# ParthaEth/GIF

Hardware: NVIDIA H100
Metric: G+D train step images/sec @256x256 bs32/GPU (higher is better)
Workload: dtype bf16x3 error-compensated tensor-core contraction (two-term bf16 operands, 3 MMAs per slice), f32 accumulate/storage

## Files before the change

### gif_b200/csrc/conv_wgrad_tc.cu

```cuda
#include <stdlib.h>

#include "tc_common.cuh"

namespace gifb200 {
namespace {

constexpr int kWgStages = 4;
constexpr int kPix = 32;
constexpr int kWgConsumerWarps = 8;
constexpr int kWgThreads = 32 * kWgConsumerWarps + 32;

struct WgParams {
    int B, Hs, Ws, Cs, Hb, Wb, Cb;
    int k, pad, s2, flip;
    int pw;
    int mr_s, mr_b;
    long long units;
    int splits;
    long long stride_t, stride_cs, stride_cb;
    long long part_stride;
};

constexpr int kHaloRows = kPix + 2;

template <int KW, int BLOCK_N, bool HALO = false, bool X3 = false, int AC = 4>
struct WgSmem {
    static constexpr int kRowBytes = X3 ? 64 : 128;
    static constexpr int kChunkBytes = kPix * kRowBytes;
    static constexpr int kHaloChunkBytes = 5120;
    static constexpr int kPlanes = X3 ? 2 : 1;
    static constexpr int kBChunks = BLOCK_N / 32;
    static constexpr int kAPlaneBytes = AC * kChunkBytes;
    static constexpr int kABytes = kPlanes * kAPlaneBytes;
    static constexpr int kBPlaneBytes = kBChunks * (HALO ? kHaloChunkBytes : kChunkBytes);
    static constexpr int kBBytesPerTap = kPlanes * kBPlaneBytes;
    static constexpr int kStages = HALO ? 5 : kWgStages;
    static constexpr int kStageBytes = HALO ? kABytes + kBBytesPerTap : kABytes + KW * kBBytesPerTap;
    static constexpr int kTxBytes = HALO ? kABytes + kPlanes * kBChunks * kHaloRows * kRowBytes : kStageBytes;
    static constexpr int kBarrierOffset = (kStages * kStageBytes + 1023) / 1024 * 1024;
    static constexpr int kDynamic = kBarrierOffset + 128 + 1024;
    static_assert(!(HALO && X3), "the halo tile is an fp32-only layout");
};

__device__ __forceinline__ uint32_t sw128_off(int row, int ch) {
    return static_cast<uint32_t>(row * 128 + ((((ch >> 2) ^ row) & 7) << 4) + (ch & 3) * 4);
}

template <int KW, int BLOCK_N, bool STACK, bool HALO, bool X3, int AC>
__global__ void __launch_bounds__(kWgThreads, 1) wgrad_tc_kernel(const __grid_constant__ CUtensorMap map_s,
                                                                 const __grid_constant__ CUtensorMap map_s2,
                                                                 const __grid_constant__ CUtensorMap map_b,
                                                                 const __grid_constant__ CUtensorMap map_b2,
                                                                 float* __restrict__ part, const WgParams p) {
    using L = WgSmem<KW, BLOCK_N, HALO, X3, AC>;
    constexpr int kM = 32 * AC;
    constexpr int kChunkBytes = L::kChunkBytes;
    constexpr int kHaloChunkBytes = L::kHaloChunkBytes;
    constexpr int kNStages = L::kStages;
    extern __shared__ uint8_t smem_raw[];
    uint8_t* smem = reinterpret_cast<uint8_t*>((reinterpret_cast<uintptr_t>(smem_raw) + 1023) & ~static_cast<uintptr_t>(1023));
    uint64_t* full_bar = reinterpret_cast<uint64_t*>(smem + L::kBarrierOffset);
    uint64_t* empty_bar = full_bar + kNStages;
    const int warp = threadIdx.x >> 5, lane = threadIdx.x & 31;

    const int ms = blockIdx.x;
    const int nb = blockIdx.y;
    const int kh = STACK ? 0 : blockIdx.z / p.splits, split = STACK ? blockIdx.z : blockIdx.z % p.splits;
    const long long per = (p.units + p.splits - 1) / p.splits;
    const long long u0 = split * per;
    const long long u1 = u0 + per < p.units ? u0 + per : p.units;
    const int iters = u1 > u0 ? static_cast<int>(u1 - u0) : 0;

    if (warp == kWgConsumerWarps && lane == 0) {
        asm volatile("prefetch.tensormap [%0];" ::"l"(&map_s) : "memory");
        asm volatile("prefetch.tensormap [%0];" ::"l"(&map_b) : "memory");
        if (X3) {
            asm volatile("prefetch.tensormap [%0];" ::"l"(&map_s2) : "memory");
            asm volatile("prefetch.tensormap [%0];" ::"l"(&map_b2) : "memory");
        }
        for (int s = 0; s < kNStages; ++s) { mbar_init(&full_bar[s], 1); mbar_init(&empty_bar[s], kWgConsumerWarps); }
        asm volatile("fence.mbarrier_init.release.cluster;" ::: "memory");
        asm volatile("fence.proxy.async.shared::cta;" ::: "memory");
    }
    __syncthreads();

    if (warp == kWgConsumerWarps) {
        if (lane == 0) {
            const int rows = kPix / p.pw;
            const int segs = p.Ws / p.pw;
            const int row_bytes = p.pw * L::kRowBytes;
            int stage = 0;
            uint32_t ph = 0;
            for (int it = 0; it < iters; ++it) {
                const long long u = u0 + it;
                mbar_wait(&empty_bar[stage], ph ^ 1);
                uint8_t* a_dst = smem + stage * L::kStageBytes;
                uint8_t* b_dst = a_dst + L::kABytes;
                mbar_expect_tx(&full_bar[stage], L::kTxBytes);
                for (int r = 0; r < rows; ++r) {
                    long long grow;
                    int x0;
                    if (rows == 1) { grow = u / segs; x0 = static_cast<int>(u % segs) * kPix; }
                    else { grow = u * rows + r; x0 = 0; }
                    const int n = static_cast<int>(grow / p.Hs), y = static_cast<int>(grow % p.Hs);
#pragma unroll
                    for (int pl = 0; pl < L::kPlanes; ++pl) {
                        const CUtensorMap* ms_ = pl ? &map_s2 : &map_s;
                        const CUtensorMap* mb_ = pl ? &map_b2 : &map_b;
                        uint8_t* a_pl = a_dst + pl * L::kAPlaneBytes;
                        if (r == 0 || !p.mr_s) {
                            for (int c = 0; c < AC; ++c) {
                                if (STACK)
                                    tma_load_4d(a_pl + c * kChunkBytes + r * row_bytes, ms_, &full_bar[stage], 0, x0,
                                                y + 1 - (c < 3 ? c : 2), n);
                                else if (AC == 2)
                                    tma_load_4d(a_pl + c * kChunkBytes + r * row_bytes, ms_, &full_bar[stage],
                                                c * 32 < p.Cs ? c * 32 : 0, x0, y, n);
                                else
                                    tma_load_4d(a_pl + c * kChunkBytes + r * row_bytes, ms_, &full_bar[stage], ms * 128 + c * 32, x0, y, n);
                            }
                        }
                        if (HALO) {
                            for (int c = 0; c < L::kBChunks; ++c)
                                tma_load_4d(b_dst + pl * L::kBPlaneBytes + c * kHaloChunkBytes, mb_, &full_bar[stage],
                                            nb * BLOCK_N + c * 32, x0 - 1, y + (STACK ? 0 : kh - p.pad), n);
                            continue;
                        }
                        if (r != 0 && p.mr_b) continue;
                        for (int kw = 0; kw < KW; ++kw)
                            for (int c = 0; c < L::kBChunks; ++c) {
                                uint8_t* dst = b_dst + kw * L::kBBytesPerTap + pl * L::kBPlaneBytes + c * kChunkBytes + r * row_bytes;
                                const int ch = nb * BLOCK_N + c * 32;
                                if (STACK)
                                    tma_load_4d(dst, mb_, &full_bar[stage], ch, x0 + kw - 1, y, n);
                                else if (!p.s2)
                                    tma_load_4d(dst, mb_, &full_bar[stage], ch, x0 + kw - p.pad, y + kh - p.pad, n);
                                else
                                    tma_load_5d(dst, mb_, &full_bar[stage], ch, kw & 1, x0 + (kw >> 1), 2 * y + kh, n);
                            }
                    }
                }
                if (++stage == kNStages) { stage = 0; ph ^= 1; }
            }
        }
        return;
    }

    float* pbase = part + split * p.part_stride;
    const int g = lane >> 2, tq = lane & 3;
    if (X3) {
        const int wg = warp >> 2, wq = warp & 3;
        constexpr int kSlices = AC == 4 ? kPix / 16 : 1;
        constexpr int kAcc = BLOCK_N / 2;
        float acc[KW][kAcc];
#pragma unroll
        for (int kw = 0; kw < KW; ++kw)
#pragma unroll
            for (int i = 0; i < kAcc; ++i) acc[kw][i] = 0.f;
        int stage = 0, prev = -1;
        uint32_t ph = 0;
        for (int it = 0; it < iters; ++it) {
            mbar_wait(&full_bar[stage], ph);
            const uint32_t a_addr = smem_u32(smem + stage * L::kStageBytes);
            const uint32_t a_row = AC == 4 ? wg * 2 * kChunkBytes : 0;
            const uint64_t adesc = make_smem_desc(a_addr + a_row, kChunkBytes, 512, 2);
            const uint64_t adesc_lo = make_smem_desc(a_addr + L::kAPlaneBytes + a_row, kChunkBytes, 512, 2);
            wgmma_fence();
#pragma unroll
            for (int kw = 0; kw < KW; ++kw) {
                fence_regs<kAcc>(acc[kw]);
                const uint32_t b_addr = a_addr + L::kABytes + kw * L::kBBytesPerTap;
                const uint64_t bdesc = make_smem_desc(b_addr, kChunkBytes, 512, 2);
                const uint64_t bdesc_lo = make_smem_desc(b_addr + L::kBPlaneBytes, kChunkBytes, 512, 2);
#pragma unroll
                for (int jj = 0; jj < kSlices; ++jj) {
                    const int j = AC == 4 ? jj : wg;
                    wgmma_bf16<BLOCK_N>(acc[kw], adesc_lo + 64 * j, bdesc + 64 * j, 1, Trans<1>());
                    wgmma_bf16<BLOCK_N>(acc[kw], adesc + 64 * j, bdesc_lo + 64 * j, 1, Trans<1>());
                    wgmma_bf16<BLOCK_N>(acc[kw], adesc + 64 * j, bdesc + 64 * j, 1, Trans<1>());
                }
            }
            wgmma_commit();
#pragma unroll
            for (int kw = 0; kw < KW; ++kw) fence_regs<kAcc>(acc[kw]);
            wgmma_wait<1>();
            if (prev >= 0 && lane == 0) mbar_arrive(&empty_bar[prev]);
            prev = stage;
            if (++stage == kNStages) { stage = 0; ph ^= 1; }
        }
        wgmma_wait<0>();
#pragma unroll
        for (int kw = 0; kw < KW; ++kw) fence_regs<kAcc>(acc[kw]);
        if constexpr (AC == 2) {
            static_assert(KW * kAcc * 128 * 4 <= kNStages * L::kStageBytes, "exchange buffer exceeds the stage ring");
            float* xch = reinterpret_cast<float*>(smem) + (threadIdx.x & 127);
            asm volatile("bar.sync 1, %0;" ::"n"(32 * kWgConsumerWarps) : "memory");
            if (wg == 1) {
#pragma unroll
                for (int kw = 0; kw < KW; ++kw)
#pragma unroll
                    for (int i = 0; i < kAcc; ++i) xch[(kw * kAcc + i) * 128] = acc[kw][i];
            }
            asm volatile("bar.sync 1, %0;" ::"n"(32 * kWgConsumerWarps) : "memory");
            if (wg == 1) return;
#pragma unroll
            for (int kw = 0; kw < KW; ++kw)
#pragma unroll
                for (int i = 0; i < kAcc; ++i) acc[kw][i] += xch[(kw * kAcc + i) * 128];
        }
#pragma unroll
        for (int h = 0; h < 2; ++h) {
            const int r = (AC == 4 ? wg * 64 : 0) + wq * 16 + g + 8 * h;
            const int q = r >> 5;
            if (STACK && q == 3) continue;
            if (AC == 2 && r >= p.Cs) continue;
            const int cs = STACK ? (r & 31) : ms * kM + r;
#pragma unroll
            for (int kw = 0; kw < KW; ++kw) {
                const int t = (STACK ? q : kh) * p.k + kw;
                float* obase = pbase + (static_cast<long long>(t) * p.Cs + cs) * p.Cb + nb * BLOCK_N + 2 * tq;
#pragma unroll
                for (int j = 0; j < BLOCK_N / 8; ++j)
                    *reinterpret_cast<float2*>(obase + 8 * j) = make_float2(acc[kw][4 * j + 2 * h], acc[kw][4 * j + 2 * h + 1]);
            }
        }
    } else {
        constexpr int kWN = kWgConsumerWarps / AC;
        const int wm = warp % AC, wn = warp / AC;
        constexpr int NT = BLOCK_N / (8 * kWN);
        float acc[KW][2][NT][4];
#pragma unroll
        for (int kw = 0; kw < KW; ++kw)
#pragma unroll
            for (int mt = 0; mt < 2; ++mt)
#pragma unroll
                for (int nt = 0; nt < NT; ++nt)
#pragma unroll
                    for (int e = 0; e < 4; ++e) acc[kw][mt][nt][e] = 0.f;
        int stage = 0;
        uint32_t ph = 0;
        for (int it = 0; it < iters; ++it) {
            mbar_wait(&full_bar[stage], ph);
            const uint8_t* sa = smem + stage * L::kStageBytes + wm * kChunkBytes;
            const uint8_t* sb = smem + stage * L::kStageBytes + L::kABytes;
#pragma unroll
            for (int k8 = 0; k8 < kPix / 8; ++k8) {
                const int k0 = k8 * 8 + tq;
                uint32_t a[2][4];
#pragma unroll
                for (int mt = 0; mt < 2; ++mt) {
                    const int ch = mt * 16 + g;
                    a[mt][0] = *reinterpret_cast<const uint32_t*>(sa + sw128_off(k0, ch));
                    a[mt][1] = *reinterpret_cast<const uint32_t*>(sa + sw128_off(k0, ch + 8));
                    a[mt][2] = *reinterpret_cast<const uint32_t*>(sa + sw128_off(k0 + 4, ch));
                    a[mt][3] = *reinterpret_cast<const uint32_t*>(sa + sw128_off(k0 + 4, ch + 8));
                }
#pragma unroll
                for (int kw = 0; kw < KW; ++kw) {
#pragma unroll
                    for (int nt = 0; nt < NT; ++nt) {
                        const int n = wn * (BLOCK_N / kWN) + nt * 8 + g;
                        const uint8_t* chunk = HALO ? sb + (n >> 5) * kHaloChunkBytes : sb + kw * L::kBBytesPerTap + (n >> 5) * kChunkBytes;
                        const int row = HALO ? k0 + kw : k0;
                        uint32_t b[2];
                        b[0] = *reinterpret_cast<const uint32_t*>(chunk + sw128_off(row, n & 31));
                        b[1] = *reinterpret_cast<const uint32_t*>(chunk + sw128_off(row + 4, n & 31));
#pragma unroll
                        for (int mt = 0; mt < 2; ++mt) mma_tf32_m16n8k8(acc[kw][mt][nt], a[mt], b);
                    }
                }
            }
            __syncwarp();
            if (lane == 0) mbar_arrive(&empty_bar[stage]);
            if (++stage == kNStages) { stage = 0; ph ^= 1; }
        }
        if (STACK && wm == 3) return;
        if (AC == 2 && wm * 32 >= p.Cs) return;
#pragma unroll
        for (int mt = 0; mt < 2; ++mt)
#pragma unroll
            for (int h = 0; h < 2; ++h) {
                const int r = wm * 32 + mt * 16 + g + 8 * h;
                const int cs = STACK ? (r & 31) : ms * kM + r;
#pragma unroll
                for (int kw = 0; kw < KW; ++kw) {
                    const int t = (STACK ? wm : kh) * p.k + kw;
                    float* obase = pbase + (static_cast<long long>(t) * p.Cs + cs) * p.Cb + nb * BLOCK_N + wn * (BLOCK_N / kWN) + 2 * tq;
#pragma unroll
                    for (int nt = 0; nt < NT; ++nt)
                        *reinterpret_cast<float2*>(obase + nt * 8) = make_float2(acc[kw][mt][nt][2 * h], acc[kw][mt][nt][2 * h + 1]);
                }
            }
    }
}

__global__ void __launch_bounds__(256) wgrad_reduce_kernel(const float* __restrict__ part, float* __restrict__ out,
                                                           WgParams p, int T) {
    const long long total = static_cast<long long>(T) * p.Cs * p.Cb;
    for (long long e = static_cast<long long>(blockIdx.x) * blockDim.x + threadIdx.x; e < total;
         e += static_cast<long long>(gridDim.x) * blockDim.x) {
        float acc = 0.f;
        for (int s = 0; s < p.splits; ++s) acc += part[s * p.part_stride + e];
        const int cb = static_cast<int>(e % p.Cb);
        const int cs = static_cast<int>((e / p.Cb) % p.Cs);
        const int t = static_cast<int>(e / (static_cast<long long>(p.Cb) * p.Cs));
        const int tt = p.flip ? T - 1 - t : t;
        out[tt * p.stride_t + cs * p.stride_cs + cb * p.stride_cb] = acc;
    }
}

inline bool pow2i(int v) { return v > 0 && (v & (v - 1)) == 0; }

int pick_bn(int Cb) {
    if (Cb % 64 == 0) return 64;
    if (Cb % 32 == 0) return 32;
    return 0;
}

struct WgMaps { CUtensorMap s, s2, b, b2; };

template <int KW, int BLOCK_N, bool STACK, bool HALO, bool X3, int AC>
int launch_wg(const WgMaps& m, float* out, float* part, const WgParams& p, cudaStream_t st) {
    using L = WgSmem<KW, BLOCK_N, HALO, X3, AC>;
    static bool attr_set = false;
    if (!attr_set) {
        cudaError_t e = cudaFuncSetAttribute(wgrad_tc_kernel<KW, BLOCK_N, STACK, HALO, X3, AC>, cudaFuncAttributeMaxDynamicSharedMemorySize, L::kDynamic);
        if (e != cudaSuccess) return fail(GIFB200_E_CUDA, "cudaFuncSetAttribute(wgrad_tc_kernel)", cudaGetErrorString(e));
        attr_set = true;
    }
    dim3 grid(STACK || AC == 2 ? 1 : p.Cs / 128, p.Cb / BLOCK_N, STACK ? p.splits : p.k * p.splits);
    wgrad_tc_kernel<KW, BLOCK_N, STACK, HALO, X3, AC><<<grid, kWgThreads, L::kDynamic, st>>>(m.s, m.s2, m.b, m.b2, part, p);
    GIFB200_LAUNCH_CHECK("wgrad_tc_kernel");
    const int T = p.k * p.k;
    const long long total = static_cast<long long>(T) * p.Cs * p.Cb;
    int blocks = cdiv(total, 256);
    if (blocks > kNumSMs * 8) blocks = kNumSMs * 8;
    wgrad_reduce_kernel<<<blocks, 256, 0, st>>>(part, out, p, T);
    GIFB200_LAUNCH_CHECK("wgrad_reduce_kernel");
    return GIFB200_OK;
}

inline bool is_stack(int Cs, int k, int mode) { return Cs == 32 && mode == 0 && k == 3; }
inline bool is_narrow(int Cs, int Cb, int k, int mode) { return Cs == 64 || (Cs == 32 && mode == 0 && k == 1 && Cb <= 64); }

void roles(int Hi, int Wi, int Ci, int Ho, int Wo, int Co, int mode, int& Hs, int& Ws, int& Cs, int& Hb, int& Wb, int& Cb) {
    if (mode == 2) { Hs = Hi; Ws = Wi; Cs = Ci; Hb = Ho; Wb = Wo; Cb = Co; }
    else { Hs = Ho; Ws = Wo; Cs = Co; Hb = Hi; Wb = Wi; Cb = Ci; }
}

}

bool conv2d_wgrad_tc_supported(int B, int Hi, int Wi, int Ci, int Ho, int Wo, int Co, int k, int mode) {
    if (B <= 0 || !(k == 3 || (k == 1 && mode == 0))) return false;
    if (mode == 0 && !(Ho == Hi && Wo == Wi)) return false;
    if (mode == 1 && !(Hi == 2 * Ho + 1 && Wi == 2 * Wo + 1)) return false;
    if (mode == 2 && !(Ho == 2 * Hi + 1 && Wo == 2 * Wi + 1)) return false;
    int Hs, Ws, Cs, Hb, Wb, Cb;
    roles(Hi, Wi, Ci, Ho, Wo, Co, mode, Hs, Ws, Cs, Hb, Wb, Cb);
    if ((Cs % 128 != 0 && !is_stack(Cs, k, mode) && !is_narrow(Cs, Cb, k, mode)) || pick_bn(Cb) == 0) return false;
    if (!pow2i(Hs) || !pow2i(Ws) || Ws < 4 || Hs < 4) return false;
    if ((static_cast<long long>(B) * Hs * Ws) % kPix != 0) return false;
    const int pw = Ws < kPix ? Ws : kPix;
    if ((static_cast<long long>(B) * Hs) % (kPix / pw) != 0) return false;
    return true;
}

static long long wgrad_splits(int B, int Hi, int Wi, int Ci, int Ho, int Wo, int Co, int k, int mode, long long* units_out) {
    int Hs, Ws, Cs, Hb, Wb, Cb;
    roles(Hi, Wi, Ci, Ho, Wo, Co, mode, Hs, Ws, Cs, Hb, Wb, Cb);
    const long long units = static_cast<long long>(B) * Hs * Ws / kPix;
    const int bn = pick_bn(Cb);
    const long long m_tiles = is_narrow(Cs, Cb, k, mode) ? 1 : Cs / 128;
    const long long base_ctas = is_stack(Cs, k, mode) ? (Cb / bn) : m_tiles * (Cb / bn) * k;
    long long splits = kNumSMs / base_ctas;
    if (splits > units) splits = units;
    if (splits < 1) splits = 1;
    if (units_out) *units_out = units;
    return splits;
}

size_t conv2d_wgrad_tc_workspace_bytes(int B, int Hi, int Wi, int Ci, int Ho, int Wo, int Co, int k, int mode) {
    if (!conv2d_wgrad_tc_supported(B, Hi, Wi, Ci, Ho, Wo, Co, k, mode)) return 0;
    return static_cast<size_t>(wgrad_splits(B, Hi, Wi, Ci, Ho, Wo, Co, k, mode, nullptr)) * k * k * Co * Ci * sizeof(float) + 256;
}

template <bool X3>
static int dispatch_wg(int k, int bn, bool stack, bool narrow, bool halo, const WgMaps& m, float* gw, float* part, const WgParams& p,
                       cudaStream_t st) {
#define GIFB200_WG(KW, BN, ST, HA) launch_wg<KW, BN, ST, HA, X3, 4>(m, gw, part, p, st)
#define GIFB200_WGN(KW, BN, HA) launch_wg<KW, BN, false, HA, X3, 2>(m, gw, part, p, st)
    if (narrow) {
        if constexpr (!X3)
            if (halo) return bn == 64 ? GIFB200_WGN(3, 64, true) : GIFB200_WGN(3, 32, true);
        if (k == 3) return bn == 64 ? GIFB200_WGN(3, 64, false) : GIFB200_WGN(3, 32, false);
        return bn == 64 ? GIFB200_WGN(1, 64, false) : GIFB200_WGN(1, 32, false);
    }
    if constexpr (!X3) {
        if (stack && halo) return bn == 64 ? GIFB200_WG(3, 64, true, true) : GIFB200_WG(3, 32, true, true);
        if (halo) return bn == 64 ? GIFB200_WG(3, 64, false, true) : GIFB200_WG(3, 32, false, true);
    }
    if (stack) return bn == 64 ? GIFB200_WG(3, 64, true, false) : GIFB200_WG(3, 32, true, false);
    if (k == 3) return bn == 64 ? GIFB200_WG(3, 64, false, false) : GIFB200_WG(3, 32, false, false);
    return bn == 64 ? GIFB200_WG(1, 64, false, false) : GIFB200_WG(1, 32, false, false);
#undef GIFB200_WGN
#undef GIFB200_WG
}

int conv2d_wgrad_tc(const float* x, const float* gy, float* gw, int B, int Hi, int Wi, int Ci, int Ho, int Wo, int Co,
                    int k, int mode, int flip, int transposed, void* ws, size_t ws_bytes, cudaStream_t st, bool x3) {
    GIFB200_REQUIRE(ws && ws_bytes >= conv2d_wgrad_tc_workspace_bytes(B, Hi, Wi, Ci, Ho, Wo, Co, k, mode), GIFB200_E_WORKSPACE,
                    "conv2d_wgrad_tc: workspace too small (see gifb200_conv2d_wgrad_workspace_bytes)");
    float* part = reinterpret_cast<float*>((reinterpret_cast<uintptr_t>(ws) + 255) & ~static_cast<uintptr_t>(255));
    GIFB200_REQUIRE(conv2d_wgrad_tc_supported(B, Hi, Wi, Ci, Ho, Wo, Co, k, mode), GIFB200_E_SHAPE,
                    "conv2d_wgrad_tc: unsupported shape");
    GIFB200_REQUIRE(aligned16(x) && aligned16(gy), GIFB200_E_ALIGN, "conv2d_wgrad_tc: x / gy must be 16-byte aligned");
    WgParams p;
    memset(&p, 0, sizeof(p));
    p.B = B; p.k = k; p.flip = flip;
    roles(Hi, Wi, Ci, Ho, Wo, Co, mode, p.Hs, p.Ws, p.Cs, p.Hb, p.Wb, p.Cb);
    const float* S = mode == 2 ? x : gy;
    const float* Bg = mode == 2 ? gy : x;
    p.s2 = mode != 0;
    p.pad = mode == 0 ? k / 2 : 0;
    p.pw = p.Ws < kPix ? p.Ws : kPix;
    p.units = static_cast<long long>(B) * p.Hs * p.Ws / kPix;
    const long long stride_o = transposed ? 1 : Ci, stride_i = transposed ? Co : 1;
    p.stride_cs = mode == 2 ? stride_i : stride_o;
    p.stride_cb = mode == 2 ? stride_o : stride_i;
    p.stride_t = static_cast<long long>(Co) * Ci;
    const int bn = pick_bn(p.Cb);
    const bool stack = is_stack(p.Cs, k, mode), narrow = is_narrow(p.Cs, p.Cb, k, mode);
    p.splits = static_cast<int>(wgrad_splits(B, Hi, Wi, Ci, Ho, Wo, Co, k, mode, nullptr));
    p.part_stride = static_cast<long long>(k) * k * Co * Ci;
    const cuuint64_t es = x3 ? 2 : 4;
    const CUtensorMapSwizzle swz = x3 ? CU_TENSOR_MAP_SWIZZLE_64B : CU_TENSOR_MAP_SWIZZLE_128B;
    const CUtensorMapDataType dt = x3 ? CU_TENSOR_MAP_DATA_TYPE_BFLOAT16 : CU_TENSOR_MAP_DATA_TYPE_FLOAT32;
    const char* Sb = reinterpret_cast<const char*>(S);
    const char* Bb = reinterpret_cast<const char*>(Bg);
    const long long s_plane = static_cast<long long>(B) * p.Hs * p.Ws * p.Cs * es;
    const long long b_plane = static_cast<long long>(B) * p.Hb * p.Wb * p.Cb * es;
    WgMaps m;
    {
        const cuuint64_t dims[4] = {static_cast<cuuint64_t>(p.Cs), static_cast<cuuint64_t>(p.Ws), static_cast<cuuint64_t>(p.Hs), static_cast<cuuint64_t>(B)};
        const cuuint64_t strides[3] = {static_cast<cuuint64_t>(p.Cs) * es, static_cast<cuuint64_t>(p.Ws) * p.Cs * es,
                                       static_cast<cuuint64_t>(p.Hs) * p.Ws * p.Cs * es};
        const int rows_per_stage = kPix / p.pw;
        const int by = rows_per_stage < p.Hs ? rows_per_stage : p.Hs, bnimg = rows_per_stage / by;
        p.mr_s = rows_per_stage > 1;
        p.mr_b = rows_per_stage > 1;
        const cuuint32_t box[4] = {32, static_cast<cuuint32_t>(p.pw), static_cast<cuuint32_t>(by), static_cast<cuuint32_t>(bnimg)};
        int rc = encode_map(&m.s, Sb, 4, dims, strides, box, swz, dt);
        if (rc == GIFB200_OK && x3) rc = encode_map(&m.s2, Sb + s_plane, 4, dims, strides, box, swz, dt);
        if (rc != GIFB200_OK) return rc;
    }
    static const int halo_env = [] { const char* e = getenv("GIFB200_WGRAD_HALO"); return e ? atoi(e) : 1; }();
    const bool halo = halo_env > 0 && !x3 && mode == 0 && k == 3 && p.pw == kPix;
    if (!p.s2) {
        const cuuint64_t dims[4] = {static_cast<cuuint64_t>(p.Cb), static_cast<cuuint64_t>(p.Wb), static_cast<cuuint64_t>(p.Hb), static_cast<cuuint64_t>(B)};
        const cuuint64_t strides[3] = {static_cast<cuuint64_t>(p.Cb) * es, static_cast<cuuint64_t>(p.Wb) * p.Cb * es,
                                       static_cast<cuuint64_t>(p.Hb) * p.Wb * p.Cb * es};
        const int rows_per_stage = kPix / p.pw;
        const int by = rows_per_stage < p.Hs ? rows_per_stage : p.Hs, bnimg = rows_per_stage / by;
        const cuuint32_t box[4] = {32, static_cast<cuuint32_t>(halo ? kHaloRows : p.pw), static_cast<cuuint32_t>(p.mr_b ? by : 1),
                                   static_cast<cuuint32_t>(p.mr_b ? bnimg : 1)};
        int rc = encode_map(&m.b, Bb, 4, dims, strides, box, swz, dt);
        if (rc == GIFB200_OK && x3) rc = encode_map(&m.b2, Bb + b_plane, 4, dims, strides, box, swz, dt);
        if (rc != GIFB200_OK) return rc;
    } else {
        const cuuint64_t dims[5] = {static_cast<cuuint64_t>(p.Cb), 2, static_cast<cuuint64_t>((p.Wb + 1) / 2), static_cast<cuuint64_t>(p.Hb), static_cast<cuuint64_t>(B)};
        const cuuint64_t strides[4] = {static_cast<cuuint64_t>(p.Cb) * es, static_cast<cuuint64_t>(p.Cb) * 2 * es,
                                       static_cast<cuuint64_t>(p.Wb) * p.Cb * es, static_cast<cuuint64_t>(p.Hb) * p.Wb * p.Cb * es};
        const int rows_per_stage = kPix / p.pw;
        const int by = rows_per_stage < p.Hs ? rows_per_stage : p.Hs, bnimg = rows_per_stage / by;
        const cuuint32_t box[5] = {32, 1, static_cast<cuuint32_t>(p.pw), static_cast<cuuint32_t>(p.mr_b ? 2 * by : 1),
                                   static_cast<cuuint32_t>(p.mr_b ? bnimg : 1)};
        const cuuint32_t estr[5] = {1, 1, 1, static_cast<cuuint32_t>(p.mr_b ? 2 : 1), 1};
        int rc = encode_map(&m.b, Bb, 5, dims, strides, box, swz, dt, estr);
        if (rc == GIFB200_OK && x3) rc = encode_map(&m.b2, Bb + b_plane, 5, dims, strides, box, swz, dt, estr);
        if (rc != GIFB200_OK) return rc;
    }
    if (!x3) { m.s2 = m.s; m.b2 = m.b; }
    return x3 ? dispatch_wg<true>(k, bn, stack, narrow, halo, m, gw, part, p, st)
              : dispatch_wg<false>(k, bn, stack, narrow, halo, m, gw, part, p, st);
}

}
```

### gif_b200/csrc/tc_common.cuh

```cuda
#pragma once
#include <cuda.h>

#include <mutex>

#include "common.cuh"

namespace gifb200 {

__device__ __forceinline__ uint32_t smem_u32(const void* p) { return static_cast<uint32_t>(__cvta_generic_to_shared(p)); }

__device__ __forceinline__ void mbar_init(uint64_t* bar, uint32_t count) {
    asm volatile("mbarrier.init.shared::cta.b64 [%0], %1;" ::"r"(smem_u32(bar)), "r"(count));
}
__device__ __forceinline__ void mbar_expect_tx(uint64_t* bar, uint32_t bytes) {
    asm volatile("mbarrier.arrive.expect_tx.shared::cta.b64 _, [%0], %1;" ::"r"(smem_u32(bar)), "r"(bytes) : "memory");
}
__device__ __forceinline__ void mbar_arrive(uint64_t* bar) {
    asm volatile("mbarrier.arrive.shared::cta.b64 _, [%0];" ::"r"(smem_u32(bar)) : "memory");
}

__device__ __forceinline__ void mbar_wait(uint64_t* bar, uint32_t parity) {
    asm volatile(
        "{\n"
        ".reg .pred p;\n"
        "WAIT_LOOP:\n"
        "mbarrier.try_wait.parity.shared::cta.b64 p, [%0], %1;\n"
        "@p bra WAIT_DONE;\n"
        "bra WAIT_LOOP;\n"
        "WAIT_DONE:\n"
        "}\n" ::"r"(smem_u32(bar)),
        "r"(parity)
        : "memory");
}
__device__ __forceinline__ void tma_load_3d(void* dst, const CUtensorMap* map, uint64_t* bar, int c0, int c1, int c2) {
    asm volatile(
        "cp.async.bulk.tensor.3d.shared::cluster.global.mbarrier::complete_tx::bytes [%0], [%1, {%3, %4, %5}], [%2];"
        ::"r"(smem_u32(dst)), "l"(map), "r"(smem_u32(bar)), "r"(c0), "r"(c1), "r"(c2)
        : "memory");
}
__device__ __forceinline__ void tma_load_4d(void* dst, const CUtensorMap* map, uint64_t* bar, int c0, int c1, int c2,
                                            int c3) {
    asm volatile(
        "cp.async.bulk.tensor.4d.shared::cluster.global.mbarrier::complete_tx::bytes [%0], [%1, {%3, %4, %5, %6}], [%2];"
        ::"r"(smem_u32(dst)), "l"(map), "r"(smem_u32(bar)), "r"(c0), "r"(c1), "r"(c2), "r"(c3)
        : "memory");
}
__device__ __forceinline__ void tma_load_5d(void* dst, const CUtensorMap* map, uint64_t* bar, int c0, int c1, int c2,
                                            int c3, int c4) {
    asm volatile(
        "cp.async.bulk.tensor.5d.shared::cluster.global.mbarrier::complete_tx::bytes [%0], [%1, {%3, %4, %5, %6, %7}], [%2];"
        ::"r"(smem_u32(dst)), "l"(map), "r"(smem_u32(bar)), "r"(c0), "r"(c1), "r"(c2), "r"(c3), "r"(c4)
        : "memory");
}
__device__ __forceinline__ void wgmma_fence() { asm volatile("wgmma.fence.sync.aligned;" ::: "memory"); }
__device__ __forceinline__ void wgmma_commit() { asm volatile("wgmma.commit_group.sync.aligned;" ::: "memory"); }
template <int N>
__device__ __forceinline__ void wgmma_wait() { asm volatile("wgmma.wait_group.sync.aligned %0;" ::"n"(N) : "memory"); }
template <int R>
__device__ __forceinline__ void setmaxnreg_inc() { asm volatile("setmaxnreg.inc.sync.aligned.u32 %0;" ::"n"(R)); }
template <int R>
__device__ __forceinline__ void setmaxnreg_dec() { asm volatile("setmaxnreg.dec.sync.aligned.u32 %0;" ::"n"(R)); }
template <int R>
__device__ __forceinline__ void fence_regs(float* d) {
#pragma unroll
    for (int i = 0; i < R; ++i) asm volatile("" : "+f"(d[i])::"memory");
}
template <int V>
struct Trans {};
template <int N>
__device__ __forceinline__ void wgmma_tf32(float* d, uint64_t da, uint64_t db, int scale_d);
template <int N, int T>
__device__ __forceinline__ void wgmma_bf16(float* d, uint64_t da, uint64_t db, int scale_d, Trans<T>);
#define GIF_F8(i) "+f"(d[i]), "+f"(d[i + 1]), "+f"(d[i + 2]), "+f"(d[i + 3]), "+f"(d[i + 4]), "+f"(d[i + 5]), "+f"(d[i + 6]), "+f"(d[i + 7])
#define GIF_F16 GIF_F8(0), GIF_F8(8)
#define GIF_F32 GIF_F16, GIF_F8(16), GIF_F8(24)
#define GIF_F64 GIF_F32, GIF_F8(32), GIF_F8(40), GIF_F8(48), GIF_F8(56)
#define GIF_R8(a, b, c, d, e, f, g, h) "%" #a ", %" #b ", %" #c ", %" #d ", %" #e ", %" #f ", %" #g ", %" #h
#define GIF_R16 GIF_R8(0, 1, 2, 3, 4, 5, 6, 7) ", " GIF_R8(8, 9, 10, 11, 12, 13, 14, 15)
#define GIF_R32 GIF_R16 ", " GIF_R8(16, 17, 18, 19, 20, 21, 22, 23) ", " GIF_R8(24, 25, 26, 27, 28, 29, 30, 31)
#define GIF_R64 GIF_R32 ", " GIF_R8(32, 33, 34, 35, 36, 37, 38, 39) ", " GIF_R8(40, 41, 42, 43, 44, 45, 46, 47) ", " \
    GIF_R8(48, 49, 50, 51, 52, 53, 54, 55) ", " GIF_R8(56, 57, 58, 59, 60, 61, 62, 63)
#define GIF_F128 GIF_F64, GIF_F8(64), GIF_F8(72), GIF_F8(80), GIF_F8(88), GIF_F8(96), GIF_F8(104), GIF_F8(112), GIF_F8(120)
#define GIF_R128 GIF_R64 ", " GIF_R8(64, 65, 66, 67, 68, 69, 70, 71) ", " GIF_R8(72, 73, 74, 75, 76, 77, 78, 79) ", " \
    GIF_R8(80, 81, 82, 83, 84, 85, 86, 87) ", " GIF_R8(88, 89, 90, 91, 92, 93, 94, 95) ", " \
    GIF_R8(96, 97, 98, 99, 100, 101, 102, 103) ", " GIF_R8(104, 105, 106, 107, 108, 109, 110, 111) ", " \
    GIF_R8(112, 113, 114, 115, 116, 117, 118, 119) ", " GIF_R8(120, 121, 122, 123, 124, 125, 126, 127)
#define GIF_WGMMA_TF32(N, R, S0, S1, S2) \
    template <> \
    __device__ __forceinline__ void wgmma_tf32<N>(float* d, uint64_t da, uint64_t db, int scale_d) { \
        asm volatile("{\n.reg .pred p;\nsetp.ne.b32 p, %" #S2 ", 0;\n" \
                     "wgmma.mma_async.sync.aligned.m64n" #N "k8.f32.tf32.tf32 {" GIF_R##R "}, %" #S0 ", %" #S1 \
                     ", p, 1, 1;\n}\n" \
                     : GIF_F##R \
                     : "l"(da), "l"(db), "r"(scale_d)); \
    }
#define GIF_WGMMA_BF16(N, R, S0, S1, S2, T0, T1, TR) \
    template <> \
    __device__ __forceinline__ void wgmma_bf16<N>(float* d, uint64_t da, uint64_t db, int scale_d, Trans<TR>) { \
        asm volatile("{\n.reg .pred p;\nsetp.ne.b32 p, %" #S2 ", 0;\n" \
                     "wgmma.mma_async.sync.aligned.m64n" #N "k16.f32.bf16.bf16 {" GIF_R##R "}, %" #S0 ", %" #S1 \
                     ", p, 1, 1, %" #T0 ", %" #T1 ";\n}\n" \
                     : GIF_F##R \
                     : "l"(da), "l"(db), "r"(scale_d), "n"(TR), "n"(TR)); \
    }
GIF_WGMMA_TF32(32, 16, 16, 17, 18)
GIF_WGMMA_TF32(64, 32, 32, 33, 34)
GIF_WGMMA_TF32(128, 64, 64, 65, 66)
GIF_WGMMA_TF32(256, 128, 128, 129, 130)
GIF_WGMMA_BF16(32, 16, 16, 17, 18, 19, 20, 0)
GIF_WGMMA_BF16(64, 32, 32, 33, 34, 35, 36, 0)
GIF_WGMMA_BF16(128, 64, 64, 65, 66, 67, 68, 0)
GIF_WGMMA_BF16(256, 128, 128, 129, 130, 131, 132, 0)
GIF_WGMMA_BF16(32, 16, 16, 17, 18, 19, 20, 1)
GIF_WGMMA_BF16(64, 32, 32, 33, 34, 35, 36, 1)

__device__ __forceinline__ void mma_tf32_m16n8k8(float* c, const uint32_t* a, const uint32_t* b) {
    asm volatile("mma.sync.aligned.m16n8k8.row.col.f32.tf32.tf32.f32 {%0, %1, %2, %3}, {%4, %5, %6, %7}, {%8, %9}, "
                 "{%0, %1, %2, %3};"
                 : "+f"(c[0]), "+f"(c[1]), "+f"(c[2]), "+f"(c[3])
                 : "r"(a[0]), "r"(a[1]), "r"(a[2]), "r"(a[3]), "r"(b[0]), "r"(b[1]));
}

__device__ __forceinline__ uint64_t make_smem_desc(uint32_t smem_addr, uint32_t lbo_bytes, uint32_t sbo_bytes, uint32_t layout) {
    uint64_t d = 0;
    d |= static_cast<uint64_t>((smem_addr & 0x3FFFF) >> 4);
    d |= static_cast<uint64_t>(lbo_bytes >> 4) << 16;
    d |= static_cast<uint64_t>(sbo_bytes >> 4) << 32;
    d |= static_cast<uint64_t>(layout) << 62;
    return d;
}
__device__ __forceinline__ uint64_t make_kmajor_sw128_desc(uint32_t smem_addr) { return make_smem_desc(smem_addr, 16, 1024, 1); }
__device__ __forceinline__ uint64_t make_kmajor_sw64_desc(uint32_t smem_addr) { return make_smem_desc(smem_addr, 16, 512, 2); }

typedef CUresult (*EncodeTiledFn)(CUtensorMap*, CUtensorMapDataType, cuuint32_t, void*, const cuuint64_t*,
                                  const cuuint64_t*, const cuuint32_t*, const cuuint32_t*, CUtensorMapInterleave,
                                  CUtensorMapSwizzle, CUtensorMapL2promotion, CUtensorMapFloatOOBfill);
inline EncodeTiledFn get_encode() {
    static EncodeTiledFn g_encode = nullptr;
    static std::once_flag g_encode_once;
    std::call_once(g_encode_once, [] {
        void* fn = nullptr;
        cudaDriverEntryPointQueryResult qres;
        if (cudaGetDriverEntryPoint("cuTensorMapEncodeTiled", &fn, cudaEnableDefault, &qres) == cudaSuccess &&
            qres == cudaDriverEntryPointSuccess)
            g_encode = reinterpret_cast<EncodeTiledFn>(fn);
    });
    return g_encode;
}

inline int encode_map(CUtensorMap* map, const void* base, int rank, const cuuint64_t* dims, const cuuint64_t* strides_bytes,
                      const cuuint32_t* box, CUtensorMapSwizzle swizzle = CU_TENSOR_MAP_SWIZZLE_128B,
                      CUtensorMapDataType dtype = CU_TENSOR_MAP_DATA_TYPE_FLOAT32, const cuuint32_t* elem_strides = nullptr) {
    EncodeTiledFn enc = get_encode();
    if (!enc) return fail(GIFB200_E_ARCH, "cuTensorMapEncodeTiled driver entry point not available");
    cuuint32_t estr[5] = {1, 1, 1, 1, 1};
    if (elem_strides)
        for (int i = 0; i < rank; ++i) estr[i] = elem_strides[i];
    CUresult r = enc(map, dtype, rank, const_cast<void*>(base), dims, strides_bytes, box, estr,
                     CU_TENSOR_MAP_INTERLEAVE_NONE, swizzle, CU_TENSOR_MAP_L2_PROMOTION_L2_256B,
                     CU_TENSOR_MAP_FLOAT_OOB_FILL_NONE);
    if (r != CUDA_SUCCESS) {
        char msg[64];
        snprintf(msg, sizeof(msg), "CUresult %d", static_cast<int>(r));
        return fail(GIFB200_E_CUDA, "cuTensorMapEncodeTiled failed", msg);
    }
    return GIFB200_OK;
}


}
```

Before: 77.25.

## Merge kw taps into one wide-N wgmma and deepen the X3 wgrad pipeline

Reorders the B stage layout so the KW taps of each plane sit next to each other. The X3 consumer can then issue one wgmma of width KW*BLOCK_N instead of KW narrower ones, which cuts instruction and descriptor overhead and lets the A operand be read once per wide MMA. The stage count for X3 is now derived from a shared-memory budget, capped at 8, rather than fixed at 4. New bf16 wgmma specialisations for N=96 and N=192 are added. The single wide accumulator array raises register pressure per thread, and the deeper ring uses more shared memory.

Measured after the change: 78.73, median of 6. 1.9% higher.

```diff
diff --git a/gif_b200/csrc/conv_wgrad_tc.cu b/gif_b200/csrc/conv_wgrad_tc.cu
--- a/gif_b200/csrc/conv_wgrad_tc.cu
+++ b/gif_b200/csrc/conv_wgrad_tc.cu
@@ -32,10 +32,10 @@
     static constexpr int kBChunks = BLOCK_N / 32;
     static constexpr int kAPlaneBytes = AC * kChunkBytes;
     static constexpr int kABytes = kPlanes * kAPlaneBytes;
-    static constexpr int kBPlaneBytes = kBChunks * (HALO ? kHaloChunkBytes : kChunkBytes);
-    static constexpr int kBBytesPerTap = kPlanes * kBPlaneBytes;
-    static constexpr int kStages = HALO ? 5 : kWgStages;
-    static constexpr int kStageBytes = HALO ? kABytes + kBBytesPerTap : kABytes + KW * kBBytesPerTap;
+    static constexpr int kBTapBytes = kBChunks * (HALO ? kHaloChunkBytes : kChunkBytes);
+    static constexpr int kBPlaneBytes = (HALO ? 1 : KW) * kBTapBytes;
+    static constexpr int kStageBytes = kABytes + kPlanes * kBPlaneBytes;
+    static constexpr int kStages = HALO ? 5 : X3 ? (225 * 1024 / kStageBytes < 8 ? 225 * 1024 / kStageBytes : 8) : kWgStages;
     static constexpr int kTxBytes = HALO ? kABytes + kPlanes * kBChunks * kHaloRows * kRowBytes : kStageBytes;
     static constexpr int kBarrierOffset = (kStages * kStageBytes + 1023) / 1024 * 1024;
     static constexpr int kDynamic = kBarrierOffset + 128 + 1024;
@@ -129,7 +129,7 @@
                         if (r != 0 && p.mr_b) continue;
                         for (int kw = 0; kw < KW; ++kw)
                             for (int c = 0; c < L::kBChunks; ++c) {
-                                uint8_t* dst = b_dst + kw * L::kBBytesPerTap + pl * L::kBPlaneBytes + c * kChunkBytes + r * row_bytes;
+                                uint8_t* dst = b_dst + pl * L::kBPlaneBytes + kw * L::kBTapBytes + c * kChunkBytes + r * row_bytes;
                                 const int ch = nb * BLOCK_N + c * 32;
                                 if (STACK)
                                     tma_load_4d(dst, mb_, &full_bar[stage], ch, x0 + kw - 1, y, n);
@@ -151,12 +151,11 @@
     if (X3) {
         const int wg = warp >> 2, wq = warp & 3;
         constexpr int kSlices = AC == 4 ? kPix / 16 : 1;
-        constexpr int kAcc = BLOCK_N / 2;
-        float acc[KW][kAcc];
-#pragma unroll
-        for (int kw = 0; kw < KW; ++kw)
-#pragma unroll
-            for (int i = 0; i < kAcc; ++i) acc[kw][i] = 0.f;
+        constexpr int kN = KW * BLOCK_N;
+        constexpr int kAcc = kN / 2;
+        float acc[kAcc];
+#pragma unroll
+        for (int i = 0; i < kAcc; ++i) acc[i] = 0.f;
         int stage = 0, prev = -1;
         uint32_t ph = 0;
         for (int it = 0; it < iters; ++it) {
@@ -166,47 +165,38 @@
             const uint64_t adesc = make_smem_desc(a_addr + a_row, kChunkBytes, 512, 2);
             const uint64_t adesc_lo = make_smem_desc(a_addr + L::kAPlaneBytes + a_row, kChunkBytes, 512, 2);
             wgmma_fence();
-#pragma unroll
-            for (int kw = 0; kw < KW; ++kw) {
-                fence_regs<kAcc>(acc[kw]);
-                const uint32_t b_addr = a_addr + L::kABytes + kw * L::kBBytesPerTap;
-                const uint64_t bdesc = make_smem_desc(b_addr, kChunkBytes, 512, 2);
-                const uint64_t bdesc_lo = make_smem_desc(b_addr + L::kBPlaneBytes, kChunkBytes, 512, 2);
-#pragma unroll
-                for (int jj = 0; jj < kSlices; ++jj) {
-                    const int j = AC == 4 ? jj : wg;
-                    wgmma_bf16<BLOCK_N>(acc[kw], adesc_lo + 64 * j, bdesc + 64 * j, 1, Trans<1>());
-                    wgmma_bf16<BLOCK_N>(acc[kw], adesc + 64 * j, bdesc_lo + 64 * j, 1, Trans<1>());
-                    wgmma_bf16<BLOCK_N>(acc[kw], adesc + 64 * j, bdesc + 64 * j, 1, Trans<1>());
-                }
+            fence_regs<kAcc>(acc);
+            const uint32_t b_addr = a_addr + L::kABytes;
+            const uint64_t bdesc = make_smem_desc(b_addr, kChunkBytes, 512, 2);
+            const uint64_t bdesc_lo = make_smem_desc(b_addr + L::kBPlaneBytes, kChunkBytes, 512, 2);
+#pragma unroll
+            for (int jj = 0; jj < kSlices; ++jj) {
+                const int j = AC == 4 ? jj : wg;
+                wgmma_bf16<kN>(acc, adesc_lo + 64 * j, bdesc + 64 * j, 1, Trans<1>());
+                wgmma_bf16<kN>(acc, adesc + 64 * j, bdesc_lo + 64 * j, 1, Trans<1>());
+                wgmma_bf16<kN>(acc, adesc + 64 * j, bdesc + 64 * j, 1, Trans<1>());
             }
             wgmma_commit();
-#pragma unroll
-            for (int kw = 0; kw < KW; ++kw) fence_regs<kAcc>(acc[kw]);
+            fence_regs<kAcc>(acc);
             wgmma_wait<1>();
             if (prev >= 0 && lane == 0) mbar_arrive(&empty_bar[prev]);
             prev = stage;
             if (++stage == kNStages) { stage = 0; ph ^= 1; }
         }
         wgmma_wait<0>();
-#pragma unroll
-        for (int kw = 0; kw < KW; ++kw) fence_regs<kAcc>(acc[kw]);
+        fence_regs<kAcc>(acc);
         if constexpr (AC == 2) {
-            static_assert(KW * kAcc * 128 * 4 <= kNStages * L::kStageBytes, "exchange buffer exceeds the stage ring");
+            static_assert(kAcc * 128 * 4 <= kNStages * L::kStageBytes, "exchange buffer exceeds the stage ring");
             float* xch = reinterpret_cast<float*>(smem) + (threadIdx.x & 127);
             asm volatile("bar.sync 1, %0;" ::"n"(32 * kWgConsumerWarps) : "memory");
             if (wg == 1) {
 #pragma unroll
-                for (int kw = 0; kw < KW; ++kw)
-#pragma unroll
-                    for (int i = 0; i < kAcc; ++i) xch[(kw * kAcc + i) * 128] = acc[kw][i];
+                for (int i = 0; i < kAcc; ++i) xch[i * 128] = acc[i];
             }
             asm volatile("bar.sync 1, %0;" ::"n"(32 * kWgConsumerWarps) : "memory");
             if (wg == 1) return;
 #pragma unroll
-            for (int kw = 0; kw < KW; ++kw)
-#pragma unroll
-                for (int i = 0; i < kAcc; ++i) acc[kw][i] += xch[(kw * kAcc + i) * 128];
+            for (int i = 0; i < kAcc; ++i) acc[i] += xch[i * 128];
         }
 #pragma unroll
         for (int h = 0; h < 2; ++h) {
@@ -220,8 +210,10 @@
                 const int t = (STACK ? q : kh) * p.k + kw;
                 float* obase = pbase + (static_cast<long long>(t) * p.Cs + cs) * p.Cb + nb * BLOCK_N + 2 * tq;
 #pragma unroll
-                for (int j = 0; j < BLOCK_N / 8; ++j)
-                    *reinterpret_cast<float2*>(obase + 8 * j) = make_float2(acc[kw][4 * j + 2 * h], acc[kw][4 * j + 2 * h + 1]);
+                for (int j = 0; j < BLOCK_N / 8; ++j) {
+                    const int f = kw * BLOCK_N / 2 + 4 * j + 2 * h;
+                    *reinterpret_cast<float2*>(obase + 8 * j) = make_float2(acc[f], acc[f + 1]);
+                }
             }
         }
     } else {
@@ -260,7 +252,7 @@
 #pragma unroll
                     for (int nt = 0; nt < NT; ++nt) {
                         const int n = wn * (BLOCK_N / kWN) + nt * 8 + g;
-                        const uint8_t* chunk = HALO ? sb + (n >> 5) * kHaloChunkBytes : sb + kw * L::kBBytesPerTap + (n >> 5) * kChunkBytes;
+                        const uint8_t* chunk = HALO ? sb + (n >> 5) * kHaloChunkBytes : sb + kw * L::kBTapBytes + (n >> 5) * kChunkBytes;
                         const int row = HALO ? k0 + kw : k0;
                         uint32_t b[2];
                         b[0] = *reinterpret_cast<const uint32_t*>(chunk + sw128_off(row, n & 31));
diff --git a/gif_b200/csrc/tc_common.cuh b/gif_b200/csrc/tc_common.cuh
--- a/gif_b200/csrc/tc_common.cuh
+++ b/gif_b200/csrc/tc_common.cuh
@@ -74,16 +74,18 @@
 #define GIF_F8(i) "+f"(d[i]), "+f"(d[i + 1]), "+f"(d[i + 2]), "+f"(d[i + 3]), "+f"(d[i + 4]), "+f"(d[i + 5]), "+f"(d[i + 6]), "+f"(d[i + 7])
 #define GIF_F16 GIF_F8(0), GIF_F8(8)
 #define GIF_F32 GIF_F16, GIF_F8(16), GIF_F8(24)
-#define GIF_F64 GIF_F32, GIF_F8(32), GIF_F8(40), GIF_F8(48), GIF_F8(56)
+#define GIF_F48 GIF_F32, GIF_F8(32), GIF_F8(40)
+#define GIF_F64 GIF_F48, GIF_F8(48), GIF_F8(56)
 #define GIF_R8(a, b, c, d, e, f, g, h) "%" #a ", %" #b ", %" #c ", %" #d ", %" #e ", %" #f ", %" #g ", %" #h
 #define GIF_R16 GIF_R8(0, 1, 2, 3, 4, 5, 6, 7) ", " GIF_R8(8, 9, 10, 11, 12, 13, 14, 15)
 #define GIF_R32 GIF_R16 ", " GIF_R8(16, 17, 18, 19, 20, 21, 22, 23) ", " GIF_R8(24, 25, 26, 27, 28, 29, 30, 31)
-#define GIF_R64 GIF_R32 ", " GIF_R8(32, 33, 34, 35, 36, 37, 38, 39) ", " GIF_R8(40, 41, 42, 43, 44, 45, 46, 47) ", " \
-    GIF_R8(48, 49, 50, 51, 52, 53, 54, 55) ", " GIF_R8(56, 57, 58, 59, 60, 61, 62, 63)
-#define GIF_F128 GIF_F64, GIF_F8(64), GIF_F8(72), GIF_F8(80), GIF_F8(88), GIF_F8(96), GIF_F8(104), GIF_F8(112), GIF_F8(120)
-#define GIF_R128 GIF_R64 ", " GIF_R8(64, 65, 66, 67, 68, 69, 70, 71) ", " GIF_R8(72, 73, 74, 75, 76, 77, 78, 79) ", " \
-    GIF_R8(80, 81, 82, 83, 84, 85, 86, 87) ", " GIF_R8(88, 89, 90, 91, 92, 93, 94, 95) ", " \
-    GIF_R8(96, 97, 98, 99, 100, 101, 102, 103) ", " GIF_R8(104, 105, 106, 107, 108, 109, 110, 111) ", " \
+#define GIF_R48 GIF_R32 ", " GIF_R8(32, 33, 34, 35, 36, 37, 38, 39) ", " GIF_R8(40, 41, 42, 43, 44, 45, 46, 47)
+#define GIF_R64 GIF_R48 ", " GIF_R8(48, 49, 50, 51, 52, 53, 54, 55) ", " GIF_R8(56, 57, 58, 59, 60, 61, 62, 63)
+#define GIF_F96 GIF_F64, GIF_F8(64), GIF_F8(72), GIF_F8(80), GIF_F8(88)
+#define GIF_F128 GIF_F96, GIF_F8(96), GIF_F8(104), GIF_F8(112), GIF_F8(120)
+#define GIF_R96 GIF_R64 ", " GIF_R8(64, 65, 66, 67, 68, 69, 70, 71) ", " GIF_R8(72, 73, 74, 75, 76, 77, 78, 79) ", " \
+    GIF_R8(80, 81, 82, 83, 84, 85, 86, 87) ", " GIF_R8(88, 89, 90, 91, 92, 93, 94, 95)
+#define GIF_R128 GIF_R96 ", " GIF_R8(96, 97, 98, 99, 100, 101, 102, 103) ", " GIF_R8(104, 105, 106, 107, 108, 109, 110, 111) ", " \
     GIF_R8(112, 113, 114, 115, 116, 117, 118, 119) ", " GIF_R8(120, 121, 122, 123, 124, 125, 126, 127)
 #define GIF_WGMMA_TF32(N, R, S0, S1, S2) \
     template <> \
@@ -113,6 +115,8 @@
 GIF_WGMMA_BF16(256, 128, 128, 129, 130, 131, 132, 0)
 GIF_WGMMA_BF16(32, 16, 16, 17, 18, 19, 20, 1)
 GIF_WGMMA_BF16(64, 32, 32, 33, 34, 35, 36, 1)
+GIF_WGMMA_BF16(96, 48, 48, 49, 50, 51, 52, 1)
+GIF_WGMMA_BF16(192, 96, 96, 97, 98, 99, 100, 1)
 
 __device__ __forceinline__ void mma_tf32_m16n8k8(float* c, const uint32_t* a, const uint32_t* b) {
     asm volatile("mma.sync.aligned.m16n8k8.row.col.f32.tf32.tf32.f32 {%0, %1, %2, %3}, {%4, %5, %6, %7}, {%8, %9}, "
```
